# zhanxw/rvtests

Measured on AMD Instinct MI355X. Metric: gene-sets/sec (SKAT+SKAT-O+CMC+Zeggini, analytic p-values), higher is better.
Workload: dtype f64

## Files before the change

### rvtests_amd/csrc/hostcheck.cpp

```cpp
#include <cstdlib>
#include <cstring>
#include <set>
#include <vector>
#include <chrono>
#include "host_stage.h"
#include "band_tiles.h"
#include "perm_counter.h"
#include "rvt_pvalue.h"
#include "rvt_mvn.h"
#include "rvt_mtscore.h"

using namespace rvt;

#ifdef RVT_DV_PROFILE
namespace rvt {
long long rvt_dv_profile[8];
std::vector<long long> g_dv_log;
void rvt_dv_eval_mark() {
  for (int k = 0; k < 5; ++k) g_dv_log.push_back(rvt_dv_profile[k]);
}
std::set<unsigned long long> g_dv_keys[2];
long long g_dv_key_calls[2];
void rvt_dv_key(int kind, double u) {
  unsigned long long b;
  std::memcpy(&b, &u, 8);
  g_dv_keys[kind].insert(b);
  ++g_dv_key_calls[kind];
}
}
// ... 341 lines not shown
}
int hc_band_tile_of(int h, int j, int W, int halo) { return rvt::band_tile_of(h, j, W, halo); }
long long hc_band_slices(int n_tiles, long long chunks, long long max_part_bytes) {
  return rvt::band_slices(n_tiles, chunks, (size_t)max_part_bytes);
}
int hc_gemm_f64_tiles(int M, int Ntot, int symmetric, int halo, int* out) {
  int nct = 0;
  const int n = rvt::gemm_f64_tiles(M, Ntot, symmetric != 0, &nct, halo);
  if (out) {
    int t = 0;
    const int nrp = (M + rvt::kGemmTileM - 1) / rvt::kGemmTileM;
    for (int rp = 0; rp < nrp; ++rp) {
      const int first = symmetric ? (rp * rvt::kGemmTileM) / rvt::kGemmTileN : 0;
      const int last = symmetric ? rvt::gemm_f64_panel_last(rp, nct, halo) : nct;
      for (int ct = first; ct < last; ++ct, ++t) {
        out[2 * t] = rp;
        out[2 * t + 1] = ct;
      }
    }
  }
  return n;
}

int hc_pack_column(const double* g, size_t n, unsigned char* out, size_t pitch, int isa, int reps, double* mu, int* has_mu,
                   long long* n_other) {
  rvt::PackedColumn r;
  for (int k = 0; k < (reps < 1 ? 1 : reps); ++k) r = rvt::pack_column_f64(g, n, out, pitch, nullptr, isa);
  *mu = r.mu;
  *has_mu = r.has_mu ? 1 : 0;
  *n_other = r.n_other;
  return r.ok ? 1 : 0;
}
int hc_pack_column_i8(const signed char* g, size_t n, unsigned char* out, size_t pitch, int isa, int reps) {
  bool ok = false;
  for (int k = 0; k < (reps < 1 ? 1 : reps); ++k) ok = rvt::pack_column_i8(g, n, out, pitch, isa);
  return ok ? 1 : 0;
}
int hc_cpu_has(int isa) {
#if defined(__x86_64__)
  if (isa == 1) return __builtin_cpu_supports("avx2") ? 1 : 0;
  if (isa == 2) return (__builtin_cpu_supports("avx512f") && __builtin_cpu_supports("bmi2")) ? 1 : 0;
#endif
  return isa == 0;
}
}
```

### rvtests_amd/csrc/k2_hardcall.hip

```cpp
#include "suffstat_hc.hip.h"

namespace rvt {

typedef void (*hc_kernel_t)(const GeneDesc*, NullTile, long long, long long, int);
static hc_kernel_t hc_kernel(int MT, int depth, int waves) {
  if (MT < 1 || MT > kHcMaxMT || depth < 1 || depth > 9 || waves < 1 || waves > 9) return nullptr;
  switch (MT * 100 + depth * 10 + waves) {
    case 124: return gene_suffstat_hc<1, 2, 4, false>;
    case 223: return gene_suffstat_hc<2, 2, 3, false>;
    case 242: return gene_suffstat_hc<2, 4, 2, false>;
    case 241: return gene_suffstat_hc_one<2, 4, false>;
    case 322: return gene_suffstat_hc<3, 2, 2, false>;
    case 331: return gene_suffstat_hc_one<3, 3, false>;
    case 422: return gene_suffstat_hc<4, 2, 2, false>;
    case 421: return gene_suffstat_hc_one<4, 2, false>;
    case 431: return gene_suffstat_hc_one<4, 3, false>;
    case 511: return gene_suffstat_hc<5, 1, 1, false>;
    case 611: return gene_suffstat_hc<6, 1, 1, false>;
    default: return nullptr;
  }
}

bool k2_hc_has_shape(int MT, int depth, int waves) { return hc_kernel(MT, depth, waves) != nullptr; }

bool k2_launch_hc(int MT, int depth, int waves, dim3 grid, hipStream_t st, const GeneDesc* d_desc, NullTile nt, long long N,
                  long long ld, int d) {
  const hc_kernel_t k = hc_kernel(MT, depth, waves);
  if (!k) return false;
  hipLaunchKernelGGL(k, grid, dim3(64), 0, st, d_desc, nt, N, ld, d);
  return true;
}

int k2_hc_any_depth(int MT) { return hc_any_depth(MT); }

void k2_launch_hc_any(unsigned classes, dim3 grid, hipStream_t st, const GeneDesc* d_desc, NullTile nt, long long N,
                      long long ld, int d) {
  hipLaunchKernelGGL((gene_suffstat_hc_any<false>), grid, dim3(64), 0, st, d_desc, nt, N, ld, d, classes);
}

void k2_launch_classify(dim3 grid, hipStream_t st, const double* G, long long N, long long ld, int M, int* flag) {
  hipLaunchKernelGGL(block_classify_kernel<0>, grid, dim3(256), 0, st, G, N, ld, M, flag);
}

}
```

### rvtests_amd/csrc/kernels.hip.h

```cpp
#pragma once
#include <hip/hip_runtime.h>
#include <float.h>
#include "rvt_pvalue.h"
#include "rvt_mvn.h"

#include "suffstat_kernels.hip.h"
#include "suffstat_hc.hip.h"
#include "suffstat_hcw.hip.h"

namespace rvt {

#if !defined(RVT_K_SPLIT) || defined(RVT_K_ENGINE)
static __global__ __launch_bounds__(64) void gene_flags_kernel(const GeneDesc* __restrict__ genes, long long N) {
  const GeneDesc gd = genes[blockIdx.x];
  if (gd.hc && gd.flags[2 * gd.MT + 1] == 0) return;
  const int tid = threadIdx.x;
  for (int base = 0; base < gd.Mp; base += 64) {
    const int j = base + tid;
    double s = 0.0, mn = INFINITY, mx = -INFINITY;
    if (j < gd.M) {
      for (int p = 0; p < gd.n_wparts; ++p) {
        const double* c = gd.colstat + (long long)p * 3 * gd.Mp;
        s += c[j];
        mn = fmin(mn, c[gd.Mp + j]);
// ... 1415 lines not shown
  __shared__ PvShared sh;
  const GeneDesc& gd = genes[genes[blockIdx.x].pv_gene];
  const int lane = threadIdx.x;
  {
    const unsigned long long* src = reinterpret_cast<const unsigned long long*>(gd.stats);
    unsigned long long* dst = reinterpret_cast<unsigned long long*>(&sh.gs);
    for (int i = lane; i < (int)(sizeof(GeneStats) / 8); i += 64) dst[i] = src[i];
  }
  __syncthreads();
  const GeneStats& gs = sh.gs;
  const int M = gd.M;
  const int Me = (M + 1) & ~1;
  double* lam_skat = reinterpret_cast<double*>(smem);
  double* lam_zimz = lam_skat + Me;
  double* ls_skat = lam_zimz + Me;
  double* ls_zimz = ls_skat + Me;
  double* fv = ls_zimz + Me;
  const WaveDaviesLds L = wave_davies_lds_carve(reinterpret_cast<char*>(fv + 42));
  rvt_gene_result* const out = gd.result;
  const int n_skat = gs.skat_nlambda, n_zimz = gs.zimz_nlambda;
  for (int i = lane; i < n_skat; i += 64) lam_skat[i] = gd.lambda[gs.skat_lambda_off + i];
  for (int i = lane; i < n_zimz; i += 64) lam_zimz[i] = gd.lambda[gs.zimz_lambda_off + i];
  __syncthreads();
  if (lane == 0) pvalue_init_result(gs, gd.gene_id, out);
  if (gs.n_poly == 0) return;
  wave_davies_sorted(lam_skat, n_skat, ls_skat, lane);
  wave_davies_sorted(lam_zimz, n_zimz, ls_zimz, lane);
  dv_memo_clear((dv_memo_p)&sh.memo, lane, 64);
  dv_memo_clear((dv_memo_p)&sh.memo_skat, lane, 64);
  __syncthreads();
  const dv_coefs lbs[2] = {(dv_coefs)lam_zimz, (dv_coefs)lam_skat};
  const dv_coefs lss[2] = {(dv_coefs)ls_zimz, (dv_coefs)ls_skat};
  const int rs[2] = {n_zimz, n_skat};
#ifdef RVT_PROF_K4
  const long long tk_a = clock64();
#endif
  double terms = 0.0;
  const bool fam = (tests & RVT_TEST_FAMSKAT) != 0;
  const bool do_skat = (tests & (RVT_TEST_SKAT | RVT_TEST_FAMSKAT)) != 0;
  const bool do_skato = (tests & RVT_TEST_SKATO) && skato_fit_ok(gs);
  const bool skato_quad = do_skato && !gs.skato_single;
  double pv_rho = 1.0;
  SkatoMoment mo;
  mo.muQ = mo.varQ = mo.df = 1.0;
  if (lane < kNRho && skato_quad) {
    mo.muQ = gs.mom_mu[lane];
    mo.varQ = gs.mom_var[lane];
// ... 275 lines not shown
```

### rvtests_amd/csrc/rvt_engine.hip

```cpp
#define RVT_K_SPLIT
#define RVT_K_ENGINE
#include "rvt_engine_int.h"
#include <chrono>
#include <functional>
#include <thread>
#include <sched.h>
#include <sys/syscall.h>
#include <unistd.h>
#include <cctype>

extern "C" {

const char* rvt_version(void) { return "rvtests_amd 0.1 (gfx950)"; }
int64_t rvt_padded_ld(int64_t N) { return (N + 15) / 16 * 16; }
const char* rvt_last_error(const rvt_ctx* ctx) { return ctx ? ctx->err.c_str() : "null context"; }
void* rvt_stream(rvt_ctx* ctx) { return ctx ? (void*)ctx->stream : nullptr; }

int rvt_init(rvt_ctx** out, int device_id) {
  if (!out) return RVT_E_INVALID;
  *out = nullptr;
  int ndev = 0;
  if (hipGetDeviceCount(&ndev) != hipSuccess || ndev <= 0) return RVT_E_NO_DEVICE;
  if (device_id < 0 || device_id >= ndev) return RVT_E_INVALID;
  if (hipSetDevice(device_id) != hipSuccess) return RVT_E_NO_DEVICE;
  rvt_ctx* c = new rvt_ctx();
  c->device = device_id;
  std::memset(&c->timing, 0, sizeof(c->timing));
  if (const char* e = getenv("RVT_HC_FUSE")) c->hc_fuse = atoi(e) != 0;
  if (const char* e = getenv("RVT_HC_CFG")) {
    for (const char* p = e; *p;) {
      int mt = 0, dp = 0, w = 0, used = 0;
      if (sscanf(p, "%d:%dx%d%n", &mt, &dp, &w, &used) != 3 || mt < 1 || mt > kHcMaxMT || !k2_hc_has_shape(mt, dp, w)) {
        fprintf(stderr, "[rvt] RVT_HC_CFG=%s: no hard-call kernel of that class, ring depth and waves per SIMD at \"%s\"\n", e, p);
        delete c;
        return RVT_E_INVALID;
      }
      c->hc_shape[mt] = {dp, w};
      p += used;
      if (*p == ',') ++p;
    }
  }
  int stage2_cus = 0;
  if (const char* e = getenv("RVT_STAGE2_CUS")) stage2_cus = atoi(e);
  hipDeviceProp_t prop;
  const bool have_prop = hipGetDeviceProperties(&prop, device_id) == hipSuccess;
  const int ncu = have_prop ? prop.multiProcessorCount : 0;
  bool masked = false;
  if (ncu >= 64 && stage2_cus < ncu && !getenv("RVT_PLAIN_STREAMS")) {
    const int words = (ncu + 31) / 32;
    std::vector<uint32_t> m1(words, 0u), m2(words, 0u);
    stage2_cus = stage2_cus > 0 ? std::max(32, stage2_cus / 32 * 32) : 0;
// ... 101 lines not shown
  c->d_nc = c->nc_buf;
  {
    const int want = 128 * 1024;
    if (hipFuncSetAttribute(reinterpret_cast<const void*>(gene_tridiag_kernel),
                            hipFuncAttributeMaxDynamicSharedMemorySize, want) == hipSuccess)
      c->eigen_lds_max = want;
    (void)hipGetLastError();
  }
  seed_rand_state(c->rand_state, 1u);
  if (const char* e = getenv("RVT_HARDCALL")) c->hc_enabled = atoi(e) != 0;
  if (const char* e = getenv("RVT_STAGE")) c->stage_on = atoi(e) != 0;
  if (const char* e = getenv("RVT_PERM_EXACT")) c->perm_exact = atoi(e) != 0;
  if (const char* e = getenv("RVT_TRACE_SUBMIT")) c->trace_submit = atoi(e) != 0;
  hipEventCreateWithFlags(&c->ev_io, hipEventDisableTiming);
  *out = c;
  return RVT_OK;
}

static void free_null(rvt_ctx* c) {
  c->d_nulltile.reset();
  c->res_buf.reset();
  c->v_buf.reset();
  c->d_X = c->d_res = c->d_rr = c->d_v = c->d_zeros = nullptr;
  c->d_hcp_xq.reset();
  c->d_hcp_scale.reset();
  c->hcp_planes_state = 0;
  c->d_nulltile_w.reset();
  c->d_vq.reset();
  c->d_dq.reset();
  c->d_xq.reset();
  c->d_xscale.reset();
  c->d_fxq.reset();
  c->fdx_ok = false;
  c->hcx_ok = false;
  c->d_null_y.reset();
  c->have_null = false;
}

static void clear_col_kind(rvt_ctx::ColKind& ck) {
  rvt_ctx::ColKind fresh;
  fresh.cols = ck.cols;
  fresh.cache_failed = ck.cache_failed;
  ck = std::move(fresh);
}

void rvt_destroy(rvt_ctx* c) {
// ... 113 lines not shown
      if (nc.binary)
        for (int64_t i = 0; i < N; ++i) s += xa[i] * v[i] * xb[i];
      else
        for (int64_t i = 0; i < N; ++i) s += xa[i] * xb[i];
      nc.C[a * d + b] = nc.C[b * d + a] = s;
    }
  if (!invert_spd(nc.C, d, nc.Cinv)) return fail(c, RVT_E_INVALID, "X'VX is singular");
  const size_t vb = sizeof(double) * (size_t)ld;
  HIP_TRY(c, c->d_nulltile.alloc(vb * (d + 2)));
  c->d_X = c->d_nulltile;
  c->d_rr = c->d_nulltile + (size_t)ld * d;
  c->d_zeros = c->d_nulltile + (size_t)ld * (d + 1);
  HIP_TRY(c, c->res_buf.alloc(vb));
  c->d_res = c->res_buf;
  HIP_TRY(c, c->v_buf.alloc(vb));
  c->d_v = c->v_buf;
  HIP_TRY(c, hipMemset(c->d_nulltile, 0, vb * (d + 2)));
  HIP_TRY(c, hipMemset(c->d_res, 0, vb));
  HIP_TRY(c, hipMemset(c->d_v, 0, vb));
  HIP_TRY(c, hipMemcpy2D(c->d_X, vb, X, sizeof(double) * (size_t)N, sizeof(double) * (size_t)N, d,
                         hipMemcpyHostToDevice));
  HIP_TRY(c, hipMemcpy(c->d_res, res, sizeof(double) * (size_t)N, hipMemcpyHostToDevice));
  HIP_TRY(c, hipMemcpy(c->d_v, v, sizeof(double) * (size_t)N, hipMemcpyHostToDevice));
  {
    std::vector<double> rr((size_t)N);
    if (nc.binary)
      for (int64_t i = 0; i < N; ++i) rr[i] = res[i] / v[i];
    else
      for (int64_t i = 0; i < N; ++i) rr[i] = res[i];
    HIP_TRY(c, hipMemcpy(c->d_rr, rr.data(), sizeof(double) * (size_t)N, hipMemcpyHostToDevice));
  }
  if (nc.binary && c->hc_enabled && d <= kHcwMaxD) {
    bool ok = true;
    for (int64_t i = 0; i < N && ok; ++i) ok = v[i] >= 0.0 && v[i] <= 0.49;
    if (ok) {
      std::vector<unsigned char> vq((size_t)ld * 8, 0);
      for (int64_t i = 0; i < N; ++i) {
        long long q = llrint(std::ldexp(v[i], 7 * kHcwPlanes));
        unsigned char* grp = vq.data() + (size_t)(i >> 2) * 32 + (size_t)(i & 3);
        for (int p = kHcwPlanes - 1; p >= 0; --p) {
          long long r = q & 127;
          if (r >= 64) r -= 128;
          q = (q - r) >> 7;
          grp[p * 4] = (unsigned char)(signed char)r;
        }
      }
// ... 1017 lines not shown
    const int nPR = (h_desc[0].MT + 3) / 4, nPC = (h_desc[0].CT + 3) / 4;
    int npanels = 0;
    for (int pr = 0; pr < nPR; ++pr) npanels += nPC - pr;
    dim3 grid(b.n_wparts, k0, npanels), block(64);
    if (nc.binary)
      k2_launch_panel_w1(grid, gst, b.d_desc, b.nd, (long long)nc.N, (long long)nc.ld, nc.d);
    else
      k2_launch_panel_w0(grid, gst, b.d_desc, b.nd, (long long)nc.N, (long long)nc.ld, nc.d);
  }
  for (int k = k0; k < b.n_gen;) {
    const int grp = suffstat_group(h_desc[k].MT, h_desc[k].CT, nc.binary != 0);
    int e = k;
    while (e < b.n_gen && suffstat_group(h_desc[e].MT, h_desc[e].CT, nc.binary != 0) == grp) ++e;
    launch_suffstat(c, gst, grp, b.d_desc + k, e - k, b.n_wparts, b.nd);
    k = e;
  }
}

static int launch_hardcall_classes(rvt_ctx* c, const Batch& b, int k, int e, hipStream_t hst) {
  const NullConsts& nc = c->nc;
  const long long N = nc.N, ld = nc.ld;
  const int d = nc.d;
  const GeneDesc *h_desc = b.h_desc, *d_desc = b.d_desc;
  const NullTile tile{c->d_nulltile, d + 2};
  unsigned fused = 0;
  int n_fused = 0, kf = e, ef = k;
  for (int g = k; g < e && c->hc_fuse; ++g) {
    const int MT = h_desc[g].MT;
    if (MT > kHcMaxMT || k2_hc_any_depth(MT) == 0 || c->hc_shape[MT].waves != 1 || c->hc_shape[MT].depth != k2_hc_any_depth(MT))
      continue;
    if (!((fused >> MT) & 1u)) ++n_fused;
    fused |= 1u << MT;
    kf = std::min(kf, g);
    ef = std::max(ef, g + 1);
  }
  if (n_fused < 2) fused = 0;
  if (fused) {
    Scope sc(c, 4, hst);
    k2_launch_hc_any(fused, dim3(b.n_wparts, ef - kf), hst, d_desc + kf, tile, N, ld, d);
  }
  for (int g = k; g < e;) {
    const int MT = h_desc[g].MT;
    int ge = g;
    while (ge < e && h_desc[ge].MT == MT) ++ge;
    if (!((fused >> MT) & 1u)) {
      Scope sc(c, 4, hst);
      const auto sh = c->hc_shape[std::min(MT, kHcMaxMT)];
      if (!k2_launch_hc(MT, sh.depth, sh.waves, dim3(b.n_wparts, ge - g), hst, d_desc + g, tile, N, ld, d))
        return fail(c, RVT_E_INVALID, "RVT_HC_CFG: no hard-call kernel of class %d with ring depth %d x %d waves per SIMD", MT,
                    sh.depth, sh.waves);
    }
    g = ge;
  }
  return RVT_OK;
}

static int launch_integer_genes(rvt_ctx* c, const Batch& b) {
  const NullConsts& nc = c->nc;
  const long long N = nc.N, ld = nc.ld;
  const int d = nc.d, n = b.n;
  const GeneDesc *h_desc = b.h_desc, *d_desc = b.d_desc;
  const bool hcx = b.caps.hcx;
  static const int planes_sw = getenv("RVT_HCP_PLANES") ? atoi(getenv("RVT_HCP_PLANES")) : 1;
  for (int k = b.n_gen; k < n;) {
    int e = k;
    const int path = h_desc[k].hc, MT = h_desc[k].MT;
    hipStream_t hst = c->k2_stream;
    if (path == kPathHardCall && !hcx && !b.caps.hcw) {
      while (e < n && h_desc[e].hc == path) ++e;
      const int rch = launch_hardcall_classes(c, b, k, e, hst);
      if (rch) return rch;
// ... 655 lines not shown
```

### rvtests_amd/csrc/rvt_engine_int.h

```cpp
#pragma once
#include <hip/hip_runtime.h>
#include <algorithm>
#include <cstdarg>
#include <cstdio>
#include <cstdlib>
#include <cstring>
#include <ctime>
#include <deque>
#include <map>
#include <string>
#include <unordered_map>
#include <thread>
#include <vector>
#include <cmath>
#include <functional>
#include "kernels.hip.h"
#include "suffstat_lat.hip.h"
#include "suffstat_hcp.hip.h"
#include "suffstat_hcx.hip.h"
#include "suffstat_fdx.hip.h"
#include "host_stage.h"

namespace rvt {
void k2_launch_group_w0(int group, dim3 grid, hipStream_t st, const GeneDesc* d_desc, const int* list, int n_wparts,
                        NullDev nd, long long N, long long ld, int d);
void k2_launch_group_w1(int group, dim3 grid, hipStream_t st, const GeneDesc* d_desc, const int* list, int n_wparts,
                        NullDev nd, long long N, long long ld, int d);
void k2_launch_panel_w0(dim3 grid, hipStream_t st, const GeneDesc* d_desc, NullDev nd, long long N, long long ld,
                        int d);
void k2_launch_panel_w1(dim3 grid, hipStream_t st, const GeneDesc* d_desc, NullDev nd, long long N, long long ld,
                        int d);
bool k2_launch_hc(int MT, int depth, int waves, dim3 grid, hipStream_t st, const GeneDesc* d_desc, NullTile nt, long long N,
                  long long ld, int d);
bool k2_hc_has_shape(int MT, int depth, int waves);
int k2_hc_any_depth(int MT);
void k2_launch_hc_any(unsigned classes, dim3 grid, hipStream_t st, const GeneDesc* d_desc, NullTile nt, long long N,
                      long long ld, int d);
void k2_launch_hcw(int MT, dim3 grid, hipStream_t st, const GeneDesc* d_desc, NullTileW nt, long long N, long long ld,
                   int d);
void k2_launch_hcx(int MT, dim3 grid, hipStream_t st, const GeneDesc* d_desc, const NullTileX& nt, long long N, long long ld,
                   int d);
void k2_launch_fdx(int MT, dim3 grid, hipStream_t st, const GeneDesc* d_desc, const NullTileF& nt, long long N, long long ld,
                   int d);
void k2_launch_lat(int MT, dim3 grid, hipStream_t st, const GeneDesc* d_desc, NullTile nt, double den, long long N,
                   long long ld, int d);
void k2_launch_hcp(int MT, dim3 grid, hipStream_t st, const GeneDesc* d_desc, NullTile nt, long long N, long long ld,
                   int d, const HcpPlanes* planes = nullptr, bool score_only = false);
void k2_launch_classify(dim3 grid, hipStream_t st, const double* G, long long N, long long ld, int M, int* flag);
}
#include "fam_kernels.hip.h"
#include "rot_gemm.hip.h"
#include "perm_kernels.hip.h"
#include "vtprice_kernels.hip.h"
#include "burdenperm_kernels.hip.h"
#include "vcf_kernels.hip.h"
#include "bgen_kernels.hip.h"
#include "jacobi_kernels.hip.h"
#include "rvt_hyper.h"

// ... 269 lines not shown
  NullConsts* d_nc = nullptr;
  double *d_X = nullptr, *d_res = nullptr, *d_rr = nullptr, *d_v = nullptr, *d_zeros = nullptr;
  DevBuf<NullConsts> nc_buf;
  DevBuf<double> d_nulltile;
  DevBuf<double> res_buf, v_buf;
  DevBuf<double> d_nulltile_w;
  DevBuf<unsigned char> d_vq;
  DevBuf<unsigned char> d_dq, d_xq;
  DevBuf<double> d_xscale;
  NullTileX hcx_tile;
  bool hcx_ok = false;
  bool reg_defer = false;
  DevBuf<unsigned char> d_fxq;
  NullTileF fdx_tile;
  bool fdx_ok = false;
  bool dosage_float = false;
  int as_threads = 256;
  bool hcx_fused = true;
  struct HcShape {
    int depth, waves;
  };
  HcShape hc_shape[kHcMaxMT + 1] = {{0, 0}, {2, 4}, {4, 1}, {3, 1}, {2, 2}, {1, 1}, {1, 1}};
  bool hc_fuse = true;
  int64_t null_ld = 0;
  int content_hint = -1;
  std::vector<std::pair<const char*, size_t>> host_reg;
  std::vector<char> host_reg_owned;
  hipEvent_t ev_reg = nullptr;
  hipStream_t reg_stream = nullptr;
  bool reg_pending = false;
  int lattice_den = 0;
  DevBuf<int> d_kind;
  bool hc_enabled = true;
  double null_beta[RVT_MAX_COV] = {};
  bool have_null_beta = false;
  DevBuf<double> d_null_y;
  DevBuf<char> d_wald_ws;
  uint64_t fam_gen = 0;
  double fam_sigma2 = 0.0;
  DevBuf<char> d_lrt_ws;
  uint64_t lrt_gen = 0;
  double lrt_ssr0 = 0.0, lrt_slog = 0.0;
  DevBuf<char> d_gg_ws;
  bool have_grammar = false;
  int64_t gg_N = 0;
  int gg_d = 0;
// ... 325 lines not shown
```

### rvtests_amd/csrc/suffstat_hc.hip.h

```cpp
#pragma once
#include <type_traits>
#include "suffstat_kernels.hip.h"

namespace rvt {

typedef int i4_t __attribute__((ext_vector_type(4)));
typedef unsigned int u4_t __attribute__((ext_vector_type(4)));

constexpr int kHcMaxMT = 6;
constexpr int kHcMaxD = 13;
constexpr int kHcStepUnit = 12;
constexpr int kHcMaxSteps = 1020;
constexpr int kHcColstatRows = 6;

constexpr int hc_pq_tiles(int MT) { return MT * MT + MT * (MT + 1) / 2; }
constexpr int hc_pq_words(int MT) { return hc_pq_tiles(MT) * 128; }
constexpr int hc_lds_words(int MT) { return hc_pq_words(MT) + 64 * MT + 4; }

struct NullTile {
  const double* base;
  int cols;
};

__device__ __forceinline__ unsigned row16_sum(unsigned h) {
  h += (unsigned)__builtin_amdgcn_update_dpp(0, (int)h, 0xB1, 0xF, 0xF, true);
  h += (unsigned)__builtin_amdgcn_update_dpp(0, (int)h, 0x4E, 0xF, 0xF, true);
  h += (unsigned)__builtin_amdgcn_update_dpp(0, (int)h, 0x141, 0xF, 0xF, true);
  h += (unsigned)__builtin_amdgcn_update_dpp(0, (int)h, 0x140, 0xF, 0xF, true);
  return h;
}

template <int MT>
struct HcStep {
  u4_t glo[MT], ghi[MT];
  u4_t xlo, xhi;
};

template <int MT, bool NT>
__device__ __forceinline__ void hc_issue(HcStep<MT>& f, const __amdgpu_buffer_rsrc_t& rg, const unsigned (&voff)[MT],
                                         const __amdgpu_buffer_rsrc_t& rx, unsigned xoff, int imm) {
#pragma unroll
  for (int c = 0; c < MT; ++c) {
    f.glo[c] = __builtin_bit_cast(u4_t, __builtin_amdgcn_raw_buffer_load_b128(rg, voff[c] + imm, 0, NT ? 2 : 0));
    f.ghi[c] = __builtin_bit_cast(u4_t, __builtin_amdgcn_raw_buffer_load_b128(rg, voff[c] + imm + 16, 0, NT ? 2 : 0));
// ... 58 lines not shown
template <bool MASKED>
__device__ __forceinline__ void hc_finish(unsigned h, const double (&xv)[4], HcBurden& bu, unsigned vmask) {
  h = row16_sum(h);
  if (MASKED) h &= vmask;
#pragma unroll
  for (int l = 0; l < 4; ++l) {
    const unsigned cz = (h >> (8 * l)) & 0xffu;
    const unsigned cc = cz ? 1u : 0u;
    bu.zz = cz * cz + bu.zz;
    bu.cnt += cc;
    bu.a_zeg = fma((double)cz, xv[l], bu.a_zeg);
    bu.a_cmc = fma((double)cc, xv[l], bu.a_cmc);
  }
}

struct HcMaskCtx {
  unsigned* oa;
  unsigned* flag;
};

template <int MT, bool MASKED>
__device__ __forceinline__ void hc_step(const HcStep<MT>& f, const int T, d4_t (&accT)[MT], unsigned (&pk)[MT][4],
                                        unsigned (&cs)[MT], const unsigned (&fx)[MT], HcBurden& bu, bool valid,
                                        unsigned vmask, unsigned& anym, const HcMaskCtx& mc) {
  double xv[4] = {hc_dbl(f.xlo[0], f.xlo[1]), hc_dbl(f.xlo[2], f.xlo[3]), hc_dbl(f.xhi[0], f.xhi[1]),
                  hc_dbl(f.xhi[2], f.xhi[3])};
  if (MASKED) {
#pragma unroll
    for (int l = 0; l < 4; ++l) xv[l] = valid ? xv[l] : 0.0;
  }
  unsigned h = 0;
#pragma unroll
  for (int c = 0; c < MT; ++c) {
    unsigned p, m;
    hc_row<MASKED>(f.glo[c], f.ghi[c], xv, accT[c], p, m, cs[c], fx[c], h, valid);
    if (m) hc_note_masked(f.glo[c], f.ghi[c], m, mc.oa + 64 * c);
    if (hc_code3(p)) __hip_atomic_fetch_or(mc.flag, 2u, __ATOMIC_RELAXED, __HIP_MEMORY_SCOPE_WORKGROUP);
    pk[c][T] = p | (m << 2);
    anym |= m;
  }
  hc_finish<MASKED>(h, xv, bu, vmask);
}

template <int MT>
__device__ __forceinline__ void hc_gram(const unsigned (&pk)[MT][4], i4_t (&accS)[MT * (MT + 1) / 2]) {
  i4_t op[MT];
#pragma unroll
  for (int c = 0; c < MT; ++c) op[c] = i4_t{(int)pk[c][0], (int)pk[c][1], (int)pk[c][2], (int)pk[c][3]};
  int t = 0;
// ... 20 lines not shown
#pragma unroll
    for (int r = 0; r < MT; ++r) {
      const i4_t a = i4_t{(int)pk[r][0], (int)pk[r][1], (int)pk[r][2], (int)pk[r][3]};
      add(r * MT + c, __builtin_amdgcn_mfma_i32_16x16x64_i8(a, mc, i4_t{0, 0, 0, 0}, 0, 0, 0));
      if (r <= c) {
        const i4_t mr = (r == c) ? mc : mask_op(r);
        add(MT * MT + r * MT - r * (r - 1) / 2 + (c - r), __builtin_amdgcn_mfma_i32_16x16x64_i8(mr, mc, i4_t{0, 0, 0, 0}, 0, 0, 0));
      }
    }
    __builtin_amdgcn_sched_barrier(0);
  }
  __hip_atomic_fetch_or(lds + hc_pq_words(MT) + 64 * MT, 1u, __ATOMIC_RELAXED, __HIP_MEMORY_SCOPE_WORKGROUP);
}

template <int MT>
__device__ __forceinline__ void hc_group_end(const unsigned (&pk)[MT][4], i4_t (&accS)[MT * (MT + 1) / 2], unsigned& anym,
                                             unsigned* lds, int lane) {
  hc_gram<MT>(pk, accS);
  if (__builtin_amdgcn_ballot_w64(anym != 0u) != 0ull) hc_gram_masked<MT>(pk, lds, lane);
  anym = 0u;
}

template <int MT, int DEPTH, bool NT>
__device__ __forceinline__ void suffstat_hc_body(const GeneDesc& gd, const NullTile& nt, long long N, long long ld,
                                                 int d, unsigned* lds) {
  const int lane = threadIdx.x & 63;
  const int v = lane & 15, q = lane >> 4;
  const int wpart = blockIdx.x;
  if (wpart >= gd.n_wparts) return;
  constexpr int kPQ = hc_pq_words(MT);
#pragma unroll 4
  for (int w = lane; w < kPQ; w += 64) lds[w] = 0u;
#pragma unroll
  for (int c = 0; c < MT; ++c) lds[kPQ + 64 * c + lane] = (lane & 2) ? 0xffffffffu : 0u;
  if (lane < 4) lds[kPQ + 64 * MT + lane] = 0u;
  const HcMaskCtx mc{lds + kPQ + 4 * v, lds + kPQ + 64 * MT};
  unsigned anym = 0u;
  const long long nsteps = ld >> 4;
  const long long s_begin = (long long)wpart * gd.steps_per_wpart;
  long long s_end = s_begin + gd.steps_per_wpart;
  if (s_end > nsteps) s_end = nsteps;
  if (s_begin >= s_end) return;
  const int M = gd.M;
  auto uniform = [](const void* p) {
    const unsigned long long a = (unsigned long long)p;
    const unsigned lo = __builtin_amdgcn_readfirstlane((unsigned)a);
    const unsigned hi = __builtin_amdgcn_readfirstlane((unsigned)(a >> 32));
    return (void*)(((unsigned long long)hi << 32) | lo);
  };
  const unsigned gbytes = (unsigned)((unsigned long long)M * (unsigned long long)ld * 8ull);
  const __amdgpu_buffer_rsrc_t rg = __builtin_amdgcn_make_buffer_rsrc(uniform(gd.G), 0, gbytes, 0x00020000);
  const unsigned xbytes = (unsigned)((unsigned long long)(d + 1) * (unsigned long long)ld * 8ull);
  const __amdgpu_buffer_rsrc_t rx = __builtin_amdgcn_make_buffer_rsrc(uniform(nt.base), 0, xbytes, 0x00020000);
  const unsigned lane_off = (unsigned)(q * 32);
  const unsigned col_bytes = (unsigned)((unsigned long long)ld * 8ull);
  unsigned vbase[MT];
#pragma unroll
  for (int c = 0; c < MT; ++c) {
    const int col = c * 16 + v;
    vbase[c] = (col < M) ? (unsigned)col * col_bytes + lane_off : 0x80000000u;
  }
  const unsigned xbase = (v <= d) ? (unsigned)v * col_bytes + lane_off : 0x80000000u;
  unsigned fx[MT];
#pragma unroll
  for (int c = 0; c < MT; ++c) fx[c] = ((gd.pflip[c] >> v) & 1) ? 0x02020202u : 0u;

  d4_t accT[MT];
  i4_t accS[MT * (MT + 1) / 2];
  unsigned cs[MT], pk[MT][4];
#pragma unroll
  for (int c = 0; c < MT; ++c) {
    accT[c] = d4_t{0.0, 0.0, 0.0, 0.0};
    cs[c] = 0;
  }
#pragma unroll
  for (int t = 0; t < MT * (MT + 1) / 2; ++t) accS[t] = i4_t{0, 0, 0, 0};
  HcBurden bu{0.0, 0.0, 0u, 0u};

  long long s = s_begin;
  const long long full = N >> 4;
  const long long s_fast_end = (s_end < full) ? s_end : full;
  constexpr int U = (DEPTH == 3) ? 12 : 4;
  const long long n_fast = (s_fast_end > s_begin) ? (s_fast_end - s_begin) / U : 0;
  if constexpr (DEPTH == 1) {
   if (n_fast > 0) {
    unsigned voff[MT];
#pragma unroll
    for (int c = 0; c < MT; ++c) voff[c] = vbase[c] + (unsigned)(s_begin * 128);
    unsigned xoff = xbase + (unsigned)(s_begin * 128);
    u4_t glo[MT], ghi[MT], xlo[2], xhi[2];
#pragma unroll
    for (int c = 0; c < MT; ++c) {
      glo[c] = __builtin_bit_cast(u4_t, __builtin_amdgcn_raw_buffer_load_b128(rg, voff[c], 0, NT ? 2 : 0));
      ghi[c] = __builtin_bit_cast(u4_t, __builtin_amdgcn_raw_buffer_load_b128(rg, voff[c] + 16, 0, NT ? 2 : 0));
    }
    xlo[0] = __builtin_bit_cast(u4_t, __builtin_amdgcn_raw_buffer_load_b128(rx, xoff, 0, 0));
    xhi[0] = __builtin_bit_cast(u4_t, __builtin_amdgcn_raw_buffer_load_b128(rx, xoff + 16, 0, 0));
    for (long long it = 0; it < n_fast; ++it) {
#pragma unroll
      for (int u = 0; u < 4; ++u) {
        xlo[(u + 1) & 1] = __builtin_bit_cast(u4_t, __builtin_amdgcn_raw_buffer_load_b128(rx, xoff + (u + 1) * 128, 0, 0));
        xhi[(u + 1) & 1] = __builtin_bit_cast(u4_t, __builtin_amdgcn_raw_buffer_load_b128(rx, xoff + (u + 1) * 128 + 16, 0, 0));
        __builtin_amdgcn_sched_barrier(0);
        const double xv[4] = {hc_dbl(xlo[u & 1][0], xlo[u & 1][1]), hc_dbl(xlo[u & 1][2], xlo[u & 1][3]),
                              hc_dbl(xhi[u & 1][0], xhi[u & 1][1]), hc_dbl(xhi[u & 1][2], xhi[u & 1][3])};
        unsigned h = 0;
#pragma unroll
        for (int c = 0; c < MT; ++c) {
          unsigned p, m;
          hc_row<false>(glo[c], ghi[c], xv, accT[c], p, m, cs[c], fx[c], h, true);
          if (m) hc_note_masked(glo[c], ghi[c], m, mc.oa + 64 * c);
          if (hc_code3(p)) __hip_atomic_fetch_or(mc.flag, 2u, __ATOMIC_RELAXED, __HIP_MEMORY_SCOPE_WORKGROUP);
          pk[c][u] = p | (m << 2);
          anym |= m;
          glo[c] = __builtin_bit_cast(u4_t, __builtin_amdgcn_raw_buffer_load_b128(rg, voff[c] + (u + 1) * 128, 0, NT ? 2 : 0));
          ghi[c] = __builtin_bit_cast(u4_t, __builtin_amdgcn_raw_buffer_load_b128(rg, voff[c] + (u + 1) * 128 + 16, 0, NT ? 2 : 0));
          __builtin_amdgcn_sched_barrier(0);
        }
        hc_finish<false>(h, xv, bu, 0xffffffffu);
        if (u == 3) hc_group_end<MT>(pk, accS, anym, lds, lane);
        __builtin_amdgcn_sched_barrier(0);
      }
#pragma unroll
      for (int c = 0; c < MT; ++c) voff[c] += 4 * 128;
      xoff += 4 * 128;
    }
    s += n_fast * U;
   }
  } else if (n_fast > 0) {
    unsigned voff[MT];
#pragma unroll
    for (int c = 0; c < MT; ++c) voff[c] = vbase[c] + (unsigned)(s_begin * 128);
    unsigned xoff = xbase + (unsigned)(s_begin * 128);
    HcStep<MT> f[DEPTH];
#pragma unroll
    for (int u = 0; u < DEPTH - 1; ++u) hc_issue<MT, NT>(f[u], rg, voff, rx, xoff, u * 128);
    for (long long it = 0; it < n_fast; ++it) {
#pragma unroll
      for (int u = 0; u < U; ++u) {
        hc_issue<MT, NT>(f[(u + DEPTH - 1) % DEPTH], rg, voff, rx, xoff, (u + DEPTH - 1) * 128);
        __builtin_amdgcn_sched_barrier(0);
        hc_step<MT, false>(f[u % DEPTH], u & 3, accT, pk, cs, fx, bu, true, 0xffffffffu, anym, mc);
        if ((u & 3) == 3) hc_group_end<MT>(pk, accS, anym, lds, lane);
        __builtin_amdgcn_sched_barrier(0);
      }
#pragma unroll
      for (int c = 0; c < MT; ++c) voff[c] += U * 128;
      xoff += U * 128;
    }
    s += n_fast * U;
  }
  while (s < s_end) {
#pragma unroll
    for (int c = 0; c < MT; ++c) pk[c][0] = pk[c][1] = pk[c][2] = pk[c][3] = 0u;
    auto one = [&](const int T, long long su) {
      const bool valid = su < s_end;
      const long long sc = valid ? su : s_end - 1;
      unsigned voff[MT];
#pragma unroll
      for (int c = 0; c < MT; ++c) voff[c] = vbase[c] + (unsigned)(sc * 128);
      HcStep<MT> f;
      hc_issue<MT, false>(f, rg, voff, rx, xbase + (unsigned)(sc * 128), 0);
      unsigned vmask = 0u;
      const long long smp = sc * 16 + q * 4;
#pragma unroll
      for (int l = 0; l < 4; ++l) vmask |= (valid && smp + l < N) ? (0xffu << (8 * l)) : 0u;
      hc_step<MT, true>(f, T, accT, pk, cs, fx, bu, valid, vmask, anym, mc);
    };
    one(0, s);
    one(1, s + 1);
    one(2, s + 2);
    one(3, s + 3);
    hc_group_end<MT>(pk, accS, anym, lds, lane);
    s += 4;
  }

  double* out = gd.parts + (long long)wpart * gd.Mp * gd.Cp;
  const int Cp = gd.Cp;
  {
    int t = 0;
#pragma unroll
    for (int r = 0; r < MT; ++r)
#pragma unroll
      for (int c = r; c < MT; ++c, ++t) {
        const int col = c * 16 + v;
        if (col < M) {
#pragma unroll
          for (int i = 0; i < 4; ++i) out[(long long)(r * 16 + q * 4 + i) * Cp + col] = (double)accS[t][i];
        }
      }
// ... 57 lines not shown
    unsigned zz = bu.zz, cn = bu.cnt;
    zz += __shfl_xor(zz, 16, 64);
    cn += __shfl_xor(cn, 16, 64);
    zz += __shfl_xor(zz, 32, 64);
    cn += __shfl_xor(cn, 32, 64);
    const int rl = 3 + d;
    double* bp = gd.bparts + (long long)wpart * 2 * rl;
    if (lane <= d) {
      const int k = (lane == d) ? 0 : 3 + lane;
      bp[k] = ac;
      bp[rl + k] = az;
    }
    if (lane == 0) {
      bp[1] = (double)cn;
      bp[2] = (double)cn;
      bp[rl + 1] = (double)zz;
      bp[rl + 2] = (double)cn;
    }
  }
}

template <int MT, int DEPTH, int WAVES, bool NT>
__global__ __launch_bounds__(64, WAVES) void gene_suffstat_hc(const GeneDesc* __restrict__ genes, NullTile nt,
                                                              long long N, long long ld, int d) {
  __shared__ unsigned lds[hc_lds_words(MT)];
  const GeneDesc gd = genes[blockIdx.y];
  if (gd.MT != MT) return;
  suffstat_hc_body<MT, DEPTH, NT>(gd, nt, N, ld, d, lds);
}

#define RVT_HC_ONE_WAVE __launch_bounds__(64) __attribute__((amdgpu_waves_per_eu(1, 1)))
template <int MT, int DEPTH, bool NT>
__global__ RVT_HC_ONE_WAVE void gene_suffstat_hc_one(const GeneDesc* __restrict__ genes, NullTile nt, long long N,
                                                     long long ld, int d) {
  __shared__ unsigned lds[hc_lds_words(MT)];
  const GeneDesc gd = genes[blockIdx.y];
  if (gd.MT != MT) return;
  suffstat_hc_body<MT, DEPTH, NT>(gd, nt, N, ld, d, lds);
}

constexpr int kHcAnyMaxMT = 5;
constexpr int hc_any_depth(int MT) { return MT == 2 ? 4 : (MT == 3 ? 3 : (MT == 4 ? 2 : (MT == 5 ? 1 : 0))); }
template <bool NT>
__global__ RVT_HC_ONE_WAVE void gene_suffstat_hc_any(const GeneDesc* __restrict__ genes, NullTile nt, long long N,
                                                              long long ld, int d, unsigned classes) {
  __shared__ unsigned lds[hc_lds_words(kHcAnyMaxMT)];
  const GeneDesc gd = genes[blockIdx.y];
  if (!((classes >> gd.MT) & 1u)) return;
  switch (gd.MT) {
    case 2: suffstat_hc_body<2, hc_any_depth(2), NT>(gd, nt, N, ld, d, lds); break;
    case 3: suffstat_hc_body<3, hc_any_depth(3), NT>(gd, nt, N, ld, d, lds); break;
    case 4: suffstat_hc_body<4, hc_any_depth(4), NT>(gd, nt, N, ld, d, lds); break;
    case 5: suffstat_hc_body<5, hc_any_depth(5), NT>(gd, nt, N, ld, d, lds); break;
    default: break;
  }
}

template <int UNUSED = 0>
__global__ __launch_bounds__(256) void block_classify_kernel(const double* __restrict__ G, long long N, long long ld,
                                                             int M, int* __restrict__ flag) {
  const long long per_col = (N + 1) / 2;
  const long long total = per_col * M;
  bool bad = false;
  for (long long idx = blockIdx.x * (long long)blockDim.x + threadIdx.x; idx < total;
       idx += (long long)gridDim.x * blockDim.x) {
    const long long j = idx / per_col, i = (idx % per_col) * 2;
    const unsigned long long* p = reinterpret_cast<const unsigned long long*>(G + j * ld + i);
    const unsigned long long a = p[0], b = (i + 1 < N) ? p[1] : 0ull;
    auto ok = [](unsigned long long x) {
      return x == 0ull || x == 0x3FF0000000000000ull || x == 0x4000000000000000ull;
    };
    bad |= !ok(a) || !ok(b);
  }
  if (__any(bad) && (threadIdx.x & 63) == 0) atomicAnd(flag, 0);
}

// ... 2 lines not shown
```

Measured before the change: 27120.

## Skip loading all-ones covariate columns and add windowed 1D hard-call grid decode

Detects covariate columns that are exactly 1.0 on the host and passes a bitmask to the hard-call kernel. Those lanes then get an out-of-range buffer offset, so the buffer loads return zero, and the value 1.0 is rebuilt by OR-ing in the high-word bits. This removes global loads for intercept columns. The launch also changes from a 2D grid to a 1D grid with an optional window that groups work-parts across genes, which changes block scheduling order. Separately, the p-value kernel now zeroes the VT result fields when analytic VT is not requested.

```diff
diff --git a/rvtests_amd/csrc/hc_window.h b/rvtests_amd/csrc/hc_window.h
--- /dev/null
+++ b/rvtests_amd/csrc/hc_window.h
@@ -0,0 +1,30 @@
+#pragma once
+
+#if defined(__HIPCC__)
+#include <hip/hip_runtime.h>
+#define RVT_HCWIN_HD __host__ __device__ inline
+#else
+#define RVT_HCWIN_HD inline
+#endif
+
+namespace rvt {
+
+struct HcGrid {
+  int P, W, genes;
+};
+
+RVT_HCWIN_HD int hc_window_of(int P, int W) { return (W >= 1 && W <= P && P % W == 0) ? W : P; }
+
+struct HcSlot {
+  int gene, wpart;
+};
+
+RVT_HCWIN_HD HcSlot hc_window_decode(unsigned id, const HcGrid& g) {
+  const unsigned W = (unsigned)hc_window_of(g.P, g.W);
+  const unsigned per_window = W * (unsigned)g.genes;
+  const unsigned w = id / per_window, r = id - w * per_window;
+  const unsigned gene = r / W;
+  return HcSlot{(int)gene, (int)(w * W + (r - gene * W))};
+}
+
+}
diff --git a/rvtests_amd/csrc/hostcheck.cpp b/rvtests_amd/csrc/hostcheck.cpp
--- a/rvtests_amd/csrc/hostcheck.cpp
+++ b/rvtests_amd/csrc/hostcheck.cpp
@@ -5,6 +5,7 @@
 #include <chrono>
 #include "host_stage.h"
 #include "band_tiles.h"
+#include "hc_window.h"
 #include "perm_counter.h"
 #include "rvt_pvalue.h"
 #include "rvt_mvn.h"
@@ -392,6 +393,16 @@
   return n;
 }
 
+int hc_hc_window_decode(int P, int W, int genes, int* out) {
+  const rvt::HcGrid g{P, W, genes};
+  for (int id = 0; id < P * genes; ++id) {
+    const rvt::HcSlot s = rvt::hc_window_decode((unsigned)id, g);
+    out[2 * id] = s.gene;
+    out[2 * id + 1] = s.wpart;
+  }
+  return rvt::hc_window_of(P, W);
+}
+
 int hc_pack_column(const double* g, size_t n, unsigned char* out, size_t pitch, int isa, int reps, double* mu, int* has_mu,
                    long long* n_other) {
   rvt::PackedColumn r;
diff --git a/rvtests_amd/csrc/k2_hardcall.hip b/rvtests_amd/csrc/k2_hardcall.hip
--- a/rvtests_amd/csrc/k2_hardcall.hip
+++ b/rvtests_amd/csrc/k2_hardcall.hip
@@ -2,7 +2,7 @@
 
 namespace rvt {
 
-typedef void (*hc_kernel_t)(const GeneDesc*, NullTile, long long, long long, int);
+typedef void (*hc_kernel_t)(const GeneDesc*, NullTile, long long, long long, int, HcGrid);
 static hc_kernel_t hc_kernel(int MT, int depth, int waves) {
   if (MT < 1 || MT > kHcMaxMT || depth < 1 || depth > 9 || waves < 1 || waves > 9) return nullptr;
   switch (MT * 100 + depth * 10 + waves) {
@@ -23,19 +23,20 @@
 
 bool k2_hc_has_shape(int MT, int depth, int waves) { return hc_kernel(MT, depth, waves) != nullptr; }
 
-bool k2_launch_hc(int MT, int depth, int waves, dim3 grid, hipStream_t st, const GeneDesc* d_desc, NullTile nt, long long N,
+bool k2_launch_hc(int MT, int depth, int waves, HcGrid hg, hipStream_t st, const GeneDesc* d_desc, NullTile nt, long long N,
                   long long ld, int d) {
   const hc_kernel_t k = hc_kernel(MT, depth, waves);
   if (!k) return false;
-  hipLaunchKernelGGL(k, grid, dim3(64), 0, st, d_desc, nt, N, ld, d);
+  hipLaunchKernelGGL(k, dim3((unsigned)hg.P * (unsigned)hg.genes), dim3(64), 0, st, d_desc, nt, N, ld, d, hg);
   return true;
 }
 
 int k2_hc_any_depth(int MT) { return hc_any_depth(MT); }
 
-void k2_launch_hc_any(unsigned classes, dim3 grid, hipStream_t st, const GeneDesc* d_desc, NullTile nt, long long N,
+void k2_launch_hc_any(unsigned classes, HcGrid hg, hipStream_t st, const GeneDesc* d_desc, NullTile nt, long long N,
                       long long ld, int d) {
-  hipLaunchKernelGGL((gene_suffstat_hc_any<false>), grid, dim3(64), 0, st, d_desc, nt, N, ld, d, classes);
+  hipLaunchKernelGGL((gene_suffstat_hc_any<false>), dim3((unsigned)hg.P * (unsigned)hg.genes), dim3(64), 0, st, d_desc, nt, N,
+                     ld, d, classes, hg);
 }
 
 void k2_launch_classify(dim3 grid, hipStream_t st, const double* G, long long N, long long ld, int M, int* flag) {
diff --git a/rvtests_amd/csrc/kernels.hip.h b/rvtests_amd/csrc/kernels.hip.h
--- a/rvtests_amd/csrc/kernels.hip.h
+++ b/rvtests_amd/csrc/kernels.hip.h
@@ -1461,7 +1461,14 @@
   for (int i = lane; i < n_skat; i += 64) lam_skat[i] = gd.lambda[gs.skat_lambda_off + i];
   for (int i = lane; i < n_zimz; i += 64) lam_zimz[i] = gd.lambda[gs.zimz_lambda_off + i];
   __syncthreads();
-  if (lane == 0) pvalue_init_result(gs, gd.gene_id, out);
+  if (lane == 0) {
+    pvalue_init_result(gs, gd.gene_id, out);
+    if (!(tests & RVT_TEST_ANALYTICVT)) {
+      out->vt_ok = out->vt_optnum = out->vt_ncutoff = 0;
+      out->vt_minmaf = out->vt_maxmaf = out->vt_optmaf = out->vt_U = out->vt_V = out->vt_stat = 0.0;
+      out->vt_p = out->vt_p_error = 0.0;
+    }
+  }
   if (gs.n_poly == 0) return;
   wave_davies_sorted(lam_skat, n_skat, ls_skat, lane);
   wave_davies_sorted(lam_zimz, n_zimz, ls_zimz, lane);
diff --git a/rvtests_amd/csrc/rvt_engine.hip b/rvtests_amd/csrc/rvt_engine.hip
--- a/rvtests_amd/csrc/rvt_engine.hip
+++ b/rvtests_amd/csrc/rvt_engine.hip
@@ -27,6 +27,8 @@
   c->device = device_id;
   std::memset(&c->timing, 0, sizeof(c->timing));
   if (const char* e = getenv("RVT_HC_FUSE")) c->hc_fuse = atoi(e) != 0;
+  if (const char* e = getenv("RVT_HC_WINDOW")) c->hc_window = std::max(0, atoi(e));
+  if (const char* e = getenv("RVT_HC_ONES")) c->hc_ones = atoi(e) != 0;
   if (const char* e = getenv("RVT_HC_CFG")) {
     for (const char* p = e; *p;) {
       int mt = 0, dp = 0, w = 0, used = 0;
@@ -174,6 +176,7 @@
   c->res_buf.reset();
   c->v_buf.reset();
   c->d_X = c->d_res = c->d_rr = c->d_v = c->d_zeros = nullptr;
+  c->null_ones = 0u;
   c->d_hcp_xq.reset();
   c->d_hcp_scale.reset();
   c->hcp_planes_state = 0;
@@ -333,6 +336,16 @@
                          hipMemcpyHostToDevice));
   HIP_TRY(c, hipMemcpy(c->d_res, res, sizeof(double) * (size_t)N, hipMemcpyHostToDevice));
   HIP_TRY(c, hipMemcpy(c->d_v, v, sizeof(double) * (size_t)N, hipMemcpyHostToDevice));
+  for (int k = 0; k < d && c->hc_ones; ++k) {
+    const double* col = X + (size_t)k * N;
+    uint64_t bits = 0;
+    int64_t i = 0;
+    for (; i < N; ++i) {
+      std::memcpy(&bits, col + i, sizeof(bits));
+      if (bits != 0x3FF0000000000000ull) break;
+    }
+    if (i == N) c->null_ones |= 1u << k;
+  }
   {
     std::vector<double> rr((size_t)N);
     if (nc.binary)
@@ -1396,7 +1409,8 @@
   const long long N = nc.N, ld = nc.ld;
   const int d = nc.d;
   const GeneDesc *h_desc = b.h_desc, *d_desc = b.d_desc;
-  const NullTile tile{c->d_nulltile, d + 2};
+  const NullTile tile{c->d_nulltile, d + 2, c->null_ones};
+  const int window = hc_window_of(b.n_wparts, c->hc_window > 0 ? c->hc_window : b.n_wparts);
   unsigned fused = 0;
   int n_fused = 0, kf = e, ef = k;
   for (int g = k; g < e && c->hc_fuse; ++g) {
@@ -1411,7 +1425,7 @@
   if (n_fused < 2) fused = 0;
   if (fused) {
     Scope sc(c, 4, hst);
-    k2_launch_hc_any(fused, dim3(b.n_wparts, ef - kf), hst, d_desc + kf, tile, N, ld, d);
+    k2_launch_hc_any(fused, HcGrid{b.n_wparts, window, ef - kf}, hst, d_desc + kf, tile, N, ld, d);
   }
   for (int g = k; g < e;) {
     const int MT = h_desc[g].MT;
@@ -1420,7 +1434,7 @@
     if (!((fused >> MT) & 1u)) {
       Scope sc(c, 4, hst);
       const auto sh = c->hc_shape[std::min(MT, kHcMaxMT)];
-      if (!k2_launch_hc(MT, sh.depth, sh.waves, dim3(b.n_wparts, ge - g), hst, d_desc + g, tile, N, ld, d))
+      if (!k2_launch_hc(MT, sh.depth, sh.waves, HcGrid{b.n_wparts, window, ge - g}, hst, d_desc + g, tile, N, ld, d))
         return fail(c, RVT_E_INVALID, "RVT_HC_CFG: no hard-call kernel of class %d with ring depth %d x %d waves per SIMD", MT,
                     sh.depth, sh.waves);
     }
diff --git a/rvtests_amd/csrc/rvt_engine_int.h b/rvtests_amd/csrc/rvt_engine_int.h
--- a/rvtests_amd/csrc/rvt_engine_int.h
+++ b/rvtests_amd/csrc/rvt_engine_int.h
@@ -30,11 +30,11 @@
                         int d);
 void k2_launch_panel_w1(dim3 grid, hipStream_t st, const GeneDesc* d_desc, NullDev nd, long long N, long long ld,
                         int d);
-bool k2_launch_hc(int MT, int depth, int waves, dim3 grid, hipStream_t st, const GeneDesc* d_desc, NullTile nt, long long N,
+bool k2_launch_hc(int MT, int depth, int waves, HcGrid hg, hipStream_t st, const GeneDesc* d_desc, NullTile nt, long long N,
                   long long ld, int d);
 bool k2_hc_has_shape(int MT, int depth, int waves);
 int k2_hc_any_depth(int MT);
-void k2_launch_hc_any(unsigned classes, dim3 grid, hipStream_t st, const GeneDesc* d_desc, NullTile nt, long long N,
+void k2_launch_hc_any(unsigned classes, HcGrid hg, hipStream_t st, const GeneDesc* d_desc, NullTile nt, long long N,
                       long long ld, int d);
 void k2_launch_hcw(int MT, dim3 grid, hipStream_t st, const GeneDesc* d_desc, NullTileW nt, long long N, long long ld,
                    int d);
@@ -350,6 +350,9 @@
   };
   HcShape hc_shape[kHcMaxMT + 1] = {{0, 0}, {2, 4}, {4, 1}, {3, 1}, {2, 2}, {1, 1}, {1, 1}};
   bool hc_fuse = true;
+  int hc_window = 0;
+  bool hc_ones = true;
+  unsigned null_ones = 0u;
   int64_t null_ld = 0;
   int content_hint = -1;
   std::vector<std::pair<const char*, size_t>> host_reg;
diff --git a/rvtests_amd/csrc/suffstat_hc.hip.h b/rvtests_amd/csrc/suffstat_hc.hip.h
--- a/rvtests_amd/csrc/suffstat_hc.hip.h
+++ b/rvtests_amd/csrc/suffstat_hc.hip.h
@@ -1,5 +1,6 @@
 #pragma once
 #include <type_traits>
+#include "hc_window.h"
 #include "suffstat_kernels.hip.h"
 
 namespace rvt {
@@ -20,6 +21,7 @@
 struct NullTile {
   const double* base;
   int cols;
+  unsigned ones = 0u;
 };
 
 __device__ __forceinline__ unsigned row16_sum(unsigned h) {
@@ -124,9 +126,9 @@
 template <int MT, bool MASKED>
 __device__ __forceinline__ void hc_step(const HcStep<MT>& f, const int T, d4_t (&accT)[MT], unsigned (&pk)[MT][4],
                                         unsigned (&cs)[MT], const unsigned (&fx)[MT], HcBurden& bu, bool valid,
-                                        unsigned vmask, unsigned& anym, const HcMaskCtx& mc) {
-  double xv[4] = {hc_dbl(f.xlo[0], f.xlo[1]), hc_dbl(f.xlo[2], f.xlo[3]), hc_dbl(f.xhi[0], f.xhi[1]),
-                  hc_dbl(f.xhi[2], f.xhi[3])};
+                                        unsigned vmask, unsigned& anym, const HcMaskCtx& mc, unsigned xone) {
+  double xv[4] = {hc_dbl(f.xlo[0], f.xlo[1] | xone), hc_dbl(f.xlo[2], f.xlo[3] | xone), hc_dbl(f.xhi[0], f.xhi[1] | xone),
+                  hc_dbl(f.xhi[2], f.xhi[3] | xone)};
   if (MASKED) {
 #pragma unroll
     for (int l = 0; l < 4; ++l) xv[l] = valid ? xv[l] : 0.0;
@@ -193,11 +195,10 @@
 }
 
 template <int MT, int DEPTH, bool NT>
-__device__ __forceinline__ void suffstat_hc_body(const GeneDesc& gd, const NullTile& nt, long long N, long long ld,
-                                                 int d, unsigned* lds) {
+__device__ __forceinline__ void suffstat_hc_body(const GeneDesc& gd, const int wpart, const NullTile& nt, long long N,
+                                                 long long ld, int d, unsigned* lds) {
   const int lane = threadIdx.x & 63;
   const int v = lane & 15, q = lane >> 4;
-  const int wpart = blockIdx.x;
   if (wpart >= gd.n_wparts) return;
   constexpr int kPQ = hc_pq_words(MT);
 #pragma unroll 4
@@ -232,6 +233,9 @@
     vbase[c] = (col < M) ? (unsigned)col * col_bytes + lane_off : 0x80000000u;
   }
   const unsigned xbase = (v <= d) ? (unsigned)v * col_bytes + lane_off : 0x80000000u;
+  const bool is_one = v < d && ((nt.ones >> v) & 1u);
+  const unsigned xfast = is_one ? 0x80000000u : xbase;
+  const unsigned xone = is_one ? 0x3FF00000u : 0u;
   unsigned fx[MT];
 #pragma unroll
   for (int c = 0; c < MT; ++c) fx[c] = ((gd.pflip[c] >> v) & 1) ? 0x02020202u : 0u;
@@ -258,7 +262,7 @@
     unsigned voff[MT];
 #pragma unroll
     for (int c = 0; c < MT; ++c) voff[c] = vbase[c] + (unsigned)(s_begin * 128);
-    unsigned xoff = xbase + (unsigned)(s_begin * 128);
+    unsigned xoff = xfast + (unsigned)(s_begin * 128);
     u4_t glo[MT], ghi[MT], xlo[2], xhi[2];
 #pragma unroll
     for (int c = 0; c < MT; ++c) {
@@ -273,8 +277,8 @@
         xlo[(u + 1) & 1] = __builtin_bit_cast(u4_t, __builtin_amdgcn_raw_buffer_load_b128(rx, xoff + (u + 1) * 128, 0, 0));
         xhi[(u + 1) & 1] = __builtin_bit_cast(u4_t, __builtin_amdgcn_raw_buffer_load_b128(rx, xoff + (u + 1) * 128 + 16, 0, 0));
         __builtin_amdgcn_sched_barrier(0);
-        const double xv[4] = {hc_dbl(xlo[u & 1][0], xlo[u & 1][1]), hc_dbl(xlo[u & 1][2], xlo[u & 1][3]),
-                              hc_dbl(xhi[u & 1][0], xhi[u & 1][1]), hc_dbl(xhi[u & 1][2], xhi[u & 1][3])};
+        const double xv[4] = {hc_dbl(xlo[u & 1][0], xlo[u & 1][1] | xone), hc_dbl(xlo[u & 1][2], xlo[u & 1][3] | xone),
+                              hc_dbl(xhi[u & 1][0], xhi[u & 1][1] | xone), hc_dbl(xhi[u & 1][2], xhi[u & 1][3] | xone)};
         unsigned h = 0;
 #pragma unroll
         for (int c = 0; c < MT; ++c) {
@@ -302,7 +306,7 @@
     unsigned voff[MT];
 #pragma unroll
     for (int c = 0; c < MT; ++c) voff[c] = vbase[c] + (unsigned)(s_begin * 128);
-    unsigned xoff = xbase + (unsigned)(s_begin * 128);
+    unsigned xoff = xfast + (unsigned)(s_begin * 128);
     HcStep<MT> f[DEPTH];
 #pragma unroll
     for (int u = 0; u < DEPTH - 1; ++u) hc_issue<MT, NT>(f[u], rg, voff, rx, xoff, u * 128);
@@ -311,7 +315,7 @@
       for (int u = 0; u < U; ++u) {
         hc_issue<MT, NT>(f[(u + DEPTH - 1) % DEPTH], rg, voff, rx, xoff, (u + DEPTH - 1) * 128);
         __builtin_amdgcn_sched_barrier(0);
-        hc_step<MT, false>(f[u % DEPTH], u & 3, accT, pk, cs, fx, bu, true, 0xffffffffu, anym, mc);
+        hc_step<MT, false>(f[u % DEPTH], u & 3, accT, pk, cs, fx, bu, true, 0xffffffffu, anym, mc, xone);
         if ((u & 3) == 3) hc_group_end<MT>(pk, accS, anym, lds, lane);
         __builtin_amdgcn_sched_barrier(0);
       }
@@ -336,7 +340,7 @@
       const long long smp = sc * 16 + q * 4;
 #pragma unroll
       for (int l = 0; l < 4; ++l) vmask |= (valid && smp + l < N) ? (0xffu << (8 * l)) : 0u;
-      hc_step<MT, true>(f, T, accT, pk, cs, fx, bu, valid, vmask, anym, mc);
+      hc_step<MT, true>(f, T, accT, pk, cs, fx, bu, valid, vmask, anym, mc, 0u);
     };
     one(0, s);
     one(1, s + 1);
@@ -440,36 +444,39 @@
 
 template <int MT, int DEPTH, int WAVES, bool NT>
 __global__ __launch_bounds__(64, WAVES) void gene_suffstat_hc(const GeneDesc* __restrict__ genes, NullTile nt,
-                                                              long long N, long long ld, int d) {
+                                                              long long N, long long ld, int d, HcGrid hg) {
   __shared__ unsigned lds[hc_lds_words(MT)];
-  const GeneDesc gd = genes[blockIdx.y];
+  const HcSlot sl = hc_window_decode(blockIdx.x, hg);
+  const GeneDesc gd = genes[sl.gene];
   if (gd.MT != MT) return;
-  suffstat_hc_body<MT, DEPTH, NT>(gd, nt, N, ld, d, lds);
+  suffstat_hc_body<MT, DEPTH, NT>(gd, sl.wpart, nt, N, ld, d, lds);
 }
 
 #define RVT_HC_ONE_WAVE __launch_bounds__(64) __attribute__((amdgpu_waves_per_eu(1, 1)))
 template <int MT, int DEPTH, bool NT>
 __global__ RVT_HC_ONE_WAVE void gene_suffstat_hc_one(const GeneDesc* __restrict__ genes, NullTile nt, long long N,
-                                                     long long ld, int d) {
+                                                     long long ld, int d, HcGrid hg) {
   __shared__ unsigned lds[hc_lds_words(MT)];
-  const GeneDesc gd = genes[blockIdx.y];
+  const HcSlot sl = hc_window_decode(blockIdx.x, hg);
+  const GeneDesc gd = genes[sl.gene];
   if (gd.MT != MT) return;
-  suffstat_hc_body<MT, DEPTH, NT>(gd, nt, N, ld, d, lds);
+  suffstat_hc_body<MT, DEPTH, NT>(gd, sl.wpart, nt, N, ld, d, lds);
 }
 
 constexpr int kHcAnyMaxMT = 5;
 constexpr int hc_any_depth(int MT) { return MT == 2 ? 4 : (MT == 3 ? 3 : (MT == 4 ? 2 : (MT == 5 ? 1 : 0))); }
 template <bool NT>
 __global__ RVT_HC_ONE_WAVE void gene_suffstat_hc_any(const GeneDesc* __restrict__ genes, NullTile nt, long long N,
-                                                              long long ld, int d, unsigned classes) {
+                                                              long long ld, int d, unsigned classes, HcGrid hg) {
   __shared__ unsigned lds[hc_lds_words(kHcAnyMaxMT)];
-  const GeneDesc gd = genes[blockIdx.y];
+  const HcSlot sl = hc_window_decode(blockIdx.x, hg);
+  const GeneDesc gd = genes[sl.gene];
   if (!((classes >> gd.MT) & 1u)) return;
   switch (gd.MT) {
-    case 2: suffstat_hc_body<2, hc_any_depth(2), NT>(gd, nt, N, ld, d, lds); break;
-    case 3: suffstat_hc_body<3, hc_any_depth(3), NT>(gd, nt, N, ld, d, lds); break;
-    case 4: suffstat_hc_body<4, hc_any_depth(4), NT>(gd, nt, N, ld, d, lds); break;
-    case 5: suffstat_hc_body<5, hc_any_depth(5), NT>(gd, nt, N, ld, d, lds); break;
+    case 2: suffstat_hc_body<2, hc_any_depth(2), NT>(gd, sl.wpart, nt, N, ld, d, lds); break;
+    case 3: suffstat_hc_body<3, hc_any_depth(3), NT>(gd, sl.wpart, nt, N, ld, d, lds); break;
+    case 4: suffstat_hc_body<4, hc_any_depth(4), NT>(gd, sl.wpart, nt, N, ld, d, lds); break;
+    case 5: suffstat_hc_body<5, hc_any_depth(5), NT>(gd, sl.wpart, nt, N, ld, d, lds); break;
     default: break;
   }
 }
```

Result: no change. 27200, median of 6 (+0.3%).
